# titus-leistner/mmlf

Measured on AMD Instinct MI355X. Metric: 96x96 EPI patches/sec fwd+bwd, bs=512, higher is better.
Workload: dtype f32 via 2 x f16 operand split (22 significant bits per operand, locally scaled; 3 MFMA passes, f32 accumulate)

## Files before the change

mmlf_amd/csrc/elementwise.hip:

```cpp
#include "common.h"
#include "row_walk.h"
#include "../../include/mmlf_hip.h"

thread_local char g_mmlf_err[512] = "";

extern "C" const char *mmlf_last_error(void) { return g_mmlf_err; }
extern "C" int mmlf_abi_version(void) { return MMLF_ABI_VERSION; }
extern "C" int64_t mmlf_amax_entries(int B, int H, int W)
{
    if (B <= 0 || H <= 0 || W <= 0) return -1;
    return amax_entries(make_grid(B, H, W));
}
extern "C" int mmlf_grid_pad_w(void) { return GRID_PAD; }
extern "C" int mmlf_grid_pad_h(void) { return GRID_PAD; }
extern "C" int mmlf_amax_head(void) { return MMLF_AMAX_HEAD; }
extern "C" int mmlf_amax_shard_stride(void) { return MMLF_AMAX_SHARD_STRIDE; }
extern "C" int64_t mmlf_grid_alloc_positions(int B, int H, int W)
{
    if (B <= 0 || H <= 0 || W <= 0) return -1;
    return grid_alloc_positions(make_grid(B, H, W));
}
extern "C" int64_t mmlf_grid_alloc_positions_k3(int B, int H, int W)
{
    if (B <= 0 || H <= 0 || W <= 0) return -1;
// ... 154 lines not shown
{
    double a = 0, b = 0;
    for (int blk = threadIdx.x; blk < nblocks; blk += 64) {
        a += partial[((size_t)blk * 2 + 0) * C + c];
        b += partial[((size_t)blk * 2 + 1) * C + c];
    }
    for (int off = 32; off > 0; off >>= 1) {
        a += __shfl_down(a, off, 64);
        b += __shfl_down(b, off, 64);
    }
    s0 = a; s1 = b;
}

__global__ __launch_bounds__(64) void bn_stats_finalize_kernel(const double *__restrict__ partial, int nblocks, int C,
                                                               double n, const float *__restrict__ gamma,
                                                               const float *__restrict__ beta, float *running_mean,
                                                               float *running_var, double momentum, double eps,
                                                               float *save_mean, float *save_invstd, float *scale,
                                                               float *shift)
{
    const int c = blockIdx.x;
    double s, ss;
    reduce_partials(partial, nblocks, C, c, s, ss);
    if (threadIdx.x != 0) return;
    const double mean = s / n;
    double var = ss / n - mean * mean;
    if (var < 0) var = 0;
    const double invstd = 1.0 / sqrt(var + eps);
    const float meanf = (float)mean, invf = (float)invstd;
    save_mean[c] = meanf;
    save_invstd[c] = invf;
    if (running_mean) {
        const double unb = n > 1 ? var * n / (n - 1) : var;
        running_mean[c] = (float)((1.0 - momentum) * running_mean[c] + momentum * mean);
        running_var[c] = (float)((1.0 - momentum) * running_var[c] + momentum * unb);
    }
    const float sc = (gamma ? gamma[c] : 1.f) * invf;
    scale[c] = sc;
    shift[c] = (beta ? beta[c] : 0.f) - meanf * sc;
}

__global__ void bn_coeffs_eval_kernel(const float *gamma, const float *beta, const float *rm, const float *rv,
                                      double eps, float *scale, float *shift, int C)
{
    const int c = blockIdx.x * blockDim.x + threadIdx.x;
    if (c >= C) return;
    const float sc = (float)((double)(gamma ? gamma[c] : 1.f) * (1.0 / sqrt((double)rv[c] + eps)));
    scale[c] = sc;
    shift[c] = fmaf(-rm[c], sc, beta ? beta[c] : 0.f);
}

__global__ __launch_bounds__(64) void bn_bwd_finalize_kernel(const double *__restrict__ partial, int nblocks, int C,
                                                             double n, const float *__restrict__ gamma,
                                                             const float *__restrict__ invstd, float *dgamma,
                                                             float *dbeta, int accumulate, float *coef)
{
    const int c = blockIdx.x;
    double sg, sgx;
    reduce_partials(partial, nblocks, C, c, sg, sgx);
    if (threadIdx.x != 0) return;
    if (dgamma) dgamma[c] = accumulate ? dgamma[c] + (float)sgx : (float)sgx;
    if (dbeta) dbeta[c] = accumulate ? dbeta[c] + (float)sg : (float)sg;
    const double k1 = (double)(gamma ? gamma[c] : 1.f) * invstd[c];
    coef[c] = (float)k1;
    coef[C + c] = (float)(k1 * sg / n);
    coef[2 * C + c] = (float)(k1 * (double)invstd[c] * sgx / n);
}

__global__ void fold_bn_kernel(const float *__restrict__ w, const float *__restrict__ b,
                               const float *__restrict__ scale, const float *__restrict__ shift,
                               float *__restrict__ w_out, float *__restrict__ b_out, int Cout, int per_co)
{
    const long long total = (long long)Cout * per_co;
    for (long long i = blockIdx.x * (long long)blockDim.x + threadIdx.x; i < total;
         i += (long long)gridDim.x * blockDim.x) {
        const int co = (int)(i / per_co);
        w_out[i] = w[i] * scale[co];
        if (i % per_co == 0) b_out[co] = fmaf(b ? b[co] : 0.f, scale[co], shift[co]);
    }
}

template <class Op>
__device__ __forceinline__ void for_each_row_pair(int cvn, int H, int W, int nrows, float *__restrict__ amax, Op op)
{
    const int P = W + GRID_PAD, R = H + GRID_PAD;
    const RowWalk w = row_walk(cvn);
    for (int row = blockIdx.x; row < nrows; row += gridDim.x) {
        const size_t base = (size_t)row * P;
        const bool row_in = grid_row_interior(row, R, H);
        float mx = 0.f;
        int x, cg;
        for (bool in = row_walk_start(w, threadIdx.x, P, x, cg); in; in = row_walk_step(w, P, x, cg))
            op(base + x, row_in && grid_pos_interior(x, W), cg, mx);
        if (amax) mmlf_amax_update_row(mx, amax, row);
    }
}

template <int MODE, int V>
__global__ __launch_bounds__(256) void bn_rows_kernel(const float *__restrict__ z, int cs_z,
                                                      const float *__restrict__ gy, int cs_gy, int c_off_gy,
                                                      const float *__restrict__ scale,
                                                      const float *__restrict__ shift,
                                                      const float *__restrict__ mean,
                                                      const float *__restrict__ coef, int C,
                                                      float *__restrict__ out, int cs_out, int c_off_out,
                                                      int C_store, int H, int W, float *__restrict__ amax, int nrows)
{
    extern __shared__ float coefs[];
    const int cvn = row_groups(C_store, V);
    const int Cpad = cvn * V;
    for (int c = threadIdx.x; c < Cpad; c += blockDim.x) {
        const bool ok = c < C;
        coefs[c] = ok ? scale[c] : 0.f;
        coefs[Cpad + c] = ok ? shift[c] : 0.f;
        if (MODE == 1) {
            coefs[2 * Cpad + c] = ok ? mean[c] : 0.f;
            coefs[3 * Cpad + c] = ok ? coef[c] : 0.f;
            coefs[4 * Cpad + c] = ok ? coef[C + c] : 0.f;
            coefs[5 * Cpad + c] = ok ? coef[2 * C + c] : 0.f;
        }
    }
    __syncthreads();
    for_each_row_pair(cvn, H, W, nrows, amax, [&](size_t q, bool interior, int cg, float &mx) {
        float o[V];
#pragma unroll
        for (int k = 0; k < V; ++k) o[k] = 0.f;
        if (interior && V * cg < C) {
            float zz[V], gg[V];
            VecIO<V>::load_nt(z + q * cs_z + V * cg, zz);
            if (MODE == 1) VecIO<V>::load_nt(gy + q * cs_gy + c_off_gy + V * cg, gg);
#pragma unroll
            for (int k = 0; k < V; ++k) {
                const int c = V * cg + k;
                const float u = fmaf(zz[k], coefs[c], coefs[Cpad + c]);
                if (MODE == 0) {
                    o[k] = fmaxf(u, 0.f);
                } else {
                    const float g = u > 0.f ? gg[k] : 0.f;
                    o[k] = coefs[3 * Cpad + c] * g - coefs[4 * Cpad + c] - coefs[5 * Cpad + c] * (zz[k] - coefs[2 * Cpad + c]);
                }
            }
        }
#pragma unroll
        for (int k = 0; k < V; ++k) mx = fmaxf(mx, fabsf(o[k]));
        float *op = out + q * cs_out + c_off_out + V * cg;
        if (V * cg + V - 1 < C_store) {
            VecIO<V>::store_nt(op, o);
        } else {
#pragma unroll
            for (int k = 0; k < V; ++k)
                if (V * cg + k < C_store) op[k] = o[k];
        }
    });
}

template <int V>
__global__ __launch_bounds__(256) void relu_slice_rows_kernel(const float *__restrict__ src, int cs_src, int c_off,
                                                              const float *__restrict__ ref, int cs_ref, int ref_off, int C,
                                                              float *__restrict__ dst, int cs_dst, int H, int W,
                                                              float *__restrict__ amax, int nrows)
{
    for_each_row_pair(cs_dst / V, H, W, nrows, amax, [&](size_t q, bool interior, int cg, float &mx) {
        float o[V];
#pragma unroll
        for (int k = 0; k < V; ++k) o[k] = 0.f;
        if (interior && V * cg < C) {
            const float *sp = src + q * cs_src + c_off + V * cg;
            const float *rp = ref + q * cs_ref + ref_off + V * cg;
            float rr[V];
            if (V * cg + V - 1 < C) {
                VecIO<V>::load_nt(sp, o);
                VecIO<V>::load_nt(rp, rr);
            } else {
#pragma unroll
                for (int k = 0; k < V; ++k) {
                    const bool in = V * cg + k < C;
                    o[k] = in ? sp[k] : 0.f;
                    rr[k] = in ? rp[k] : 0.f;
                }
            }
#pragma unroll
            for (int k = 0; k < V; ++k) o[k] = rr[k] > 0.f ? o[k] : 0.f;
        }
#pragma unroll
        for (int k = 0; k < V; ++k) mx = fmaxf(mx, fabsf(o[k]));
        VecIO<V>::store_nt(dst + q * cs_dst + V * cg, o);
    });
}

struct BnApply4 { const float *z[4]; const float *scale[4]; const float *shift[4]; };
__global__ __launch_bounds__(256) void bn_apply4_kernel(BnApply4 s, int cs_z, int C, float *__restrict__ out,
                                                        int H, int W, float *__restrict__ amax, int nrows)
{
    extern __shared__ float coefs[];
    const int C4 = 4 * C, half = C / 2;
    for (int c = threadIdx.x; c < C4; c += blockDim.x) {
        const int k = c / C, cl = c - k * C;
        const float *sc = k == 0 ? s.scale[0] : k == 1 ? s.scale[1] : k == 2 ? s.scale[2] : s.scale[3];
        const float *sh = k == 0 ? s.shift[0] : k == 1 ? s.shift[1] : k == 2 ? s.shift[2] : s.shift[3];
        coefs[c] = sc[cl];
        coefs[C4 + c] = sh[cl];
    }
    __syncthreads();
    for_each_row_pair(2 * C, H, W, nrows, amax, [&](size_t q, bool interior, int g, float &mx) {
        float2 o = make_float2(0.f, 0.f);
        if (interior) {
            const int k = g / half, cl = 2 * (g - k * half);
            const float *zp = k == 0 ? s.z[0] : k == 1 ? s.z[1] : k == 2 ? s.z[2] : s.z[3];
            const float2 zz = *reinterpret_cast<const float2 *>(zp + q * cs_z + cl);
            o.x = fmaxf(fmaf(zz.x, coefs[2 * g], coefs[C4 + 2 * g]), 0.f);
            o.y = fmaxf(fmaf(zz.y, coefs[2 * g + 1], coefs[C4 + 2 * g + 1]), 0.f);
        }
        mx = fmaxf(mx, fmaxf(o.x, o.y));
        *reinterpret_cast<float2 *>(out + q * C4 + 2 * g) = o;
    });
}


__global__ __launch_bounds__(256) void pack_nchw_kernel(const float *__restrict__ src, int C,
                                                        float *__restrict__ grid, int cs, int H, int W,
                                                        float *__restrict__ amax, int xt)
{
    extern __shared__ float tile[];
    float mx = 0.f;
    const int P = W + GRID_PAD, R = H + GRID_PAD;
    const int row = blockIdx.x;
    const int b = row / R, y = row - b * R;
    const size_t base = (size_t)row * P;
    const int c4n = cs / 4;
    const int pitch = xt | 1;
    const bool row_in = (y >= 1 && y <= H);
    for (int x0 = 0; x0 < P; x0 += xt) {
        const int nx = min(xt, P - x0);
        for (int e = threadIdx.x; e < cs * nx; e += blockDim.x) {
            const int c = e / nx, x = x0 + e - c * nx;
            float v = 0.f;
            if (row_in && x >= 1 && x <= W && c < C) v = src[(((size_t)b * C + c) * H + (y - 1)) * W + (x - 1)];
            tile[c * pitch + (x - x0)] = v;
        }
        __syncthreads();
        for (int e = threadIdx.x; e < nx * c4n; e += blockDim.x) {
            const int xl = e / c4n, cg = e - xl * c4n;
            const float4 o = make_float4(tile[(4 * cg) * pitch + xl], tile[(4 * cg + 1) * pitch + xl],
                                         tile[(4 * cg + 2) * pitch + xl], tile[(4 * cg + 3) * pitch + xl]);
            mx = fmaxf(fmaxf(mx, fmaxf(fabsf(o.x), fabsf(o.y))), fmaxf(fabsf(o.z), fabsf(o.w)));
            *reinterpret_cast<float4 *>(grid + (base + x0 + xl) * cs + 4 * cg) = o;
        }
        __syncthreads();
    }
    if (amax) mmlf_amax_update_row(mx, amax, row);
}

__global__ __launch_bounds__(256) void unpack_nchw_kernel(const float *__restrict__ grid, int cs,
                                                          float *__restrict__ dst, int C, int H, int W, int xt)
{
    extern __shared__ float tile[];
    const int P = W + GRID_PAD, R = H + GRID_PAD;
    const int row = blockIdx.x;
    const int b = row / H, y = row - b * H + 1;
    const size_t base = ((size_t)(b * R + y)) * P;
    const int pitch = C | 1;
    for (int x0 = 0; x0 < W; x0 += xt) {
        const int nx = min(xt, W - x0);
        for (int e = threadIdx.x; e < nx * C; e += blockDim.x) {
            const int xl = e / C, c = e - xl * C;
            tile[xl * pitch + c] = grid[(base + x0 + xl + 1) * cs + c];
        }
        __syncthreads();
        for (int e = threadIdx.x; e < C * nx; e += blockDim.x) {
            const int c = e / nx, xl = e - c * nx;
            dst[(((size_t)b * C + c) * H + (y - 1)) * W + x0 + xl] = tile[xl * pitch + c];
        }
        __syncthreads();
    }
}

__device__ __forceinline__ float laplace_pdf(float x, float mu, float b)
{
    const float a = __fdiv_rn(1.0f, __fmul_rn(2.0f, b));
    const float t = __fdiv_rn(-fabsf(__fsub_rn(x, mu)), b);
    return __fmul_rn(a, expf(t));
}

__global__ void head_upr_kernel(const float *__restrict__ out, const float *__restrict__ grid,
                                float *__restrict__ post, int steps, int HW, long long total)
{
    for (long long idx = blockIdx.x * (long long)blockDim.x + threadIdx.x; idx < total;
         idx += (long long)gridDim.x * blockDim.x) {
        const long long b = idx / HW;
        const int p = (int)(idx - b * HW);
        const float mu = out[(b * 2 + 0) * HW + p];
        const float bb = expf(out[(b * 2 + 1) * HW + p]);
        for (int k = 0; k < steps; ++k) post[(b * steps + k) * HW + p] = laplace_pdf(grid[k], mu, bb);
    }
}

__global__ void head_dpp_kernel(const float *__restrict__ sc, const float *__restrict__ gt, const float *__restrict__ gn,
                                float *__restrict__ one_hot, float *__restrict__ post, float *__restrict__ mean,
                                float *__restrict__ logvar, int steps, int HW, long long total)
{
    for (long long idx = blockIdx.x * (long long)blockDim.x + threadIdx.x; idx < total;
         idx += (long long)gridDim.x * blockDim.x) {
        const long long b = idx / HW;
        const int p = (int)(idx - b * HW);
        const float *s = sc + b * steps * HW + p;
        float mx = -INFINITY, z = 0.f;
// ... 674 lines not shown
        const int p = (int)(idx - b * HW);
        float best = INFINITY;
        int bi = 0;
        for (int j = 0; j < S; ++j) {
            const float lv = logvars[(size_t)j * total + idx];
            if (lv < best) { best = lv; bi = j; }
        }
        mean[idx] = means[(size_t)bi * total + idx];
        logvar[idx] = best;
        for (int k = 0; k < S; ++k) {
            const float gk = grid[k];
            float acc = 0.f;
            for (int j = 0; j < S; ++j)
                acc = __fadd_rn(acc, laplace_pdf(gk, means[(size_t)j * total + idx],
                                                 expf(logvars[(size_t)j * total + idx])));
            post[(b * S + k) * HW + p] = __fdiv_rn(acc, (float)S);
        }
    }
}

__device__ __forceinline__ double cdf_laplace_f64(double x, double m, double v)
{
    const double z = (x - m) / v;
    return x < m ? exp(z) / 2.0 : 1.0 - exp(-z) / 2.0;
}

__global__ void lmm_to_discrete_kernel(const float *__restrict__ means, const float *__restrict__ logvars,
                                       const double *__restrict__ edges, double *__restrict__ out, int S, int B,
                                       int n_bins, long long HW)
{
    const long long total = (long long)B * n_bins * HW;
    for (long long idx = blockIdx.x * (long long)blockDim.x + threadIdx.x; idx < total;
         idx += (long long)gridDim.x * blockDim.x) {
        const long long p = idx % HW;
        const long long r = idx / HW;
        const int k = (int)(r % n_bins);
        const long long b = r / n_bins;
        const double e0 = edges[k], e1 = edges[k + 1];
        double acc = 0.0;
        for (int s = 0; s < S; ++s) {
            const size_t o = ((size_t)s * B + b) * HW + p;
            const double m = (double)means[o];
            const double v = (double)expf(logvars[o]);
            acc += cdf_laplace_f64(e1, m, v) - cdf_laplace_f64(e0, m, v);
        }
        out[idx] = acc / (double)S;
    }
}

static int ew_blocks(long long total, int per = 256)
{
    long long b = (total + per - 1) / per;
    if (b > 8192) b = 8192;
    if (b < 1) b = 1;
    return (int)b;
}

extern "C" int mmlf_bn_stats_train(const float *z, int cs, int C, const float *gamma, const float *beta,
                                   float *running_mean, float *running_var, double momentum, double eps,
                                   float *save_mean, float *save_invstd, float *scale, float *shift,
                                   double *partial, int nblocks, int B, int H, int W, void *stream)
{
    MMLF_CHECK_ARG(z && save_mean && save_invstd && scale && shift && partial, "mmlf_bn_stats_train: null pointer");
    MMLF_CHECK_ARG(cs % 4 == 0 && C > 0 && C <= cs && (C + 3) / 4 <= 256, "mmlf_bn_stats_train: C=%d cs=%d", C, cs);
    MMLF_CHECK_ARG(nblocks > 0 && nblocks <= 4096, "mmlf_bn_stats_train: nblocks=%d", nblocks);
    MMLF_CHECK_ARG(B > 0 && H > 0 && W > 0, "mmlf_bn_stats_train: bad shape B=%d H=%d W=%d", B, H, W);
    hipStream_t st = (hipStream_t)stream;
    hipLaunchKernelGGL((bn_reduce_kernel<4>), dim3(nblocks), dim3(256), 0, st, z, cs, nullptr, 0, 0, nullptr,
                       nullptr, nullptr, nullptr, C, partial, B, H, W);
    const double n = (double)B * H * W;
    hipLaunchKernelGGL(bn_stats_finalize_kernel, dim3(C), dim3(64), 0, st, partial, nblocks, C, n, gamma,
                       beta, running_mean, running_var, momentum, eps, save_mean, save_invstd, scale, shift);
    return mmlf_launch_status("mmlf_bn_stats_train");
}

extern "C" int mmlf_bn_stats_finalize(const double *partial, int nblocks, int C, const float *gamma,
                                      const float *beta, float *running_mean, float *running_var, double momentum,
                                      double eps, float *save_mean, float *save_invstd, float *scale, float *shift,
                                      int B, int H, int W, void *stream)
{
    MMLF_CHECK_ARG(partial && save_mean && save_invstd && scale && shift && C > 0 && nblocks > 0,
                   "mmlf_bn_stats_finalize: bad argument");
    MMLF_CHECK_ARG(B > 0 && H > 0 && W > 0, "mmlf_bn_stats_finalize: bad shape B=%d H=%d W=%d", B, H, W);
    hipLaunchKernelGGL(bn_stats_finalize_kernel, dim3(C), dim3(64), 0, (hipStream_t)stream, partial, nblocks, C,
                       (double)B * H * W, gamma, beta, running_mean, running_var, momentum, eps, save_mean,
                       save_invstd, scale, shift);
    return mmlf_launch_status("mmlf_bn_stats_finalize");
}

extern "C" int mmlf_bn_coeffs_eval(const float *gamma, const float *beta, const float *rm, const float *rv,
                                   double eps, float *scale, float *shift, int C, void *stream)
{
    MMLF_CHECK_ARG(rm && rv && scale && shift && C > 0, "mmlf_bn_coeffs_eval: bad argument");
    hipLaunchKernelGGL(bn_coeffs_eval_kernel, dim3((C + 63) / 64), dim3(64), 0, (hipStream_t)stream, gamma, beta, rm,
                       rv, eps, scale, shift, C);
    return mmlf_launch_status("mmlf_bn_coeffs_eval");
}

static int fold_bn_eval(const char *who, int taps, const float *w_oihw, const float *bias, const float *scale,
                        const float *shift, float *w_out, float *bias_out, int Cout, int Cin, void *stream)
{
    MMLF_CHECK_ARG(w_oihw && scale && shift && w_out && bias_out && Cout > 0 && Cin > 0, "%s: bad argument", who);
    const long long total = (long long)Cout * Cin * taps;
    hipLaunchKernelGGL(fold_bn_kernel, dim3(ew_blocks(total)), dim3(256), 0, (hipStream_t)stream, w_oihw, bias, scale,
                       shift, w_out, bias_out, Cout, Cin * taps);
    return mmlf_launch_status(who);
}

extern "C" int mmlf_fold_bn_eval(const float *w_oihw, const float *bias, const float *scale, const float *shift,
                                 float *w_out, float *bias_out, int Cout, int Cin, void *stream)
{
    return fold_bn_eval("mmlf_fold_bn_eval", 4, w_oihw, bias, scale, shift, w_out, bias_out, Cout, Cin, stream);
}

extern "C" int mmlf_fold_bn_eval3x3(const float *w_oihw, const float *bias, const float *scale, const float *shift,
                                    float *w_out, float *bias_out, int Cout, int Cin, void *stream)
{
    return fold_bn_eval("mmlf_fold_bn_eval3x3", 9, w_oihw, bias, scale, shift, w_out, bias_out, Cout, Cin, stream);
}

extern "C" int mmlf_bn_apply_relu(const float *z, int cs_z, int C, const float *scale, const float *shift, float *y,
                                  int cs_y, int c_off, int C_store, int B, int H, int W, float *amax_out,
                                  void *stream)
{
    MMLF_CHECK_ARG(z && scale && shift && y, "mmlf_bn_apply_relu: null pointer");
    MMLF_CHECK_ARG(cs_z % 4 == 0 && cs_y % 2 == 0 && c_off % 2 == 0 && c_off >= 0 && C > 0 && C <= cs_z && C_store >= C &&
                       c_off + C_store <= cs_y,
                   "mmlf_bn_apply_relu: C=%d cs_z=%d cs_y=%d c_off=%d C_store=%d", C, cs_z, cs_y, c_off, C_store);
    MMLF_CHECK_ARG(B > 0 && H > 0 && W > 0, "mmlf_bn_apply_relu: bad shape B=%d H=%d W=%d", B, H, W);
    const int nrows = B * (H + GRID_PAD);
    hipLaunchKernelGGL((bn_rows_kernel<0, 4>), dim3(nrows), dim3(256), 6 * (C_store + 4) * sizeof(float), (hipStream_t)stream, z, cs_z,
                       nullptr, 0, 0, scale, shift, nullptr, nullptr, C, y, cs_y, c_off, C_store, H, W, amax_out, nrows);
    return mmlf_launch_status("mmlf_bn_apply_relu");
}

extern "C" int mmlf_bn_apply_relu4(const float *const z[4], int cs_z, int C, const float *const scale[4],
                                   const float *const shift[4], float *y, int cs_y, int B, int H, int W,
                                   float *amax_out, void *stream)
{
    MMLF_CHECK_ARG(z && scale && shift && y && B > 0 && H > 0 && W > 0, "mmlf_bn_apply_relu4: bad argument");
    MMLF_CHECK_ARG(C > 0 && C % 2 == 0 && C <= cs_z && cs_z % 2 == 0 && cs_y == 4 * C && 8 * C * sizeof(float) <= 48 * 1024,
                   "mmlf_bn_apply_relu4: C=%d cs_z=%d cs_y=%d (needs even C, cs_y == 4 * C)", C, cs_z, cs_y);
    BnApply4 s;
    for (int k = 0; k < 4; ++k) {
        MMLF_CHECK_ARG(z[k] && scale[k] && shift[k], "mmlf_bn_apply_relu4: null pointer in source %d", k);
        s.z[k] = z[k]; s.scale[k] = scale[k]; s.shift[k] = shift[k];
    }
    const int nrows = B * (H + GRID_PAD);
    hipLaunchKernelGGL(bn_apply4_kernel, dim3(nrows), dim3(256), 8 * C * sizeof(float), (hipStream_t)stream, s, cs_z, C,
                       y, H, W, amax_out, nrows);
    return mmlf_launch_status("mmlf_bn_apply_relu4");
}

extern "C" int mmlf_bn_bwd_reduce(const float *gy, int cs_gy, int c_off, const float *z, int cs_z, int C,
                                  const float *scale, const float *shift, const float *gamma,
                                  const float *save_mean, const float *save_invstd, float *dgamma, float *dbeta,
                                  int accumulate, float *coef, double *partial, int nblocks, int B, int H, int W,
                                  void *stream)
{
    MMLF_CHECK_ARG(gy && z && scale && shift && save_mean && save_invstd && coef && partial,
                   "mmlf_bn_bwd_reduce: null pointer");
    MMLF_CHECK_ARG(cs_gy % 2 == 0 && c_off % 2 == 0 && c_off >= 0 && cs_z % 4 == 0 && C > 0 && C <= cs_z &&
                       c_off + C <= cs_gy && (C + 3) / 4 <= 128,
                   "mmlf_bn_bwd_reduce: layout C=%d cs_z=%d cs_gy=%d c_off=%d", C, cs_z, cs_gy, c_off);
    MMLF_CHECK_ARG(nblocks > 0 && nblocks <= 4096, "mmlf_bn_bwd_reduce: nblocks=%d", nblocks);
    MMLF_CHECK_ARG(B > 0 && H > 0 && W > 0, "mmlf_bn_bwd_reduce: bad shape B=%d H=%d W=%d", B, H, W);
    hipStream_t st = (hipStream_t)stream;
    hipLaunchKernelGGL(bn_reduce_bwd_kernel, dim3(nblocks), dim3(256), 0, st, z, cs_z, gy, cs_gy, c_off,
                       scale, shift, save_mean, save_invstd, C, partial, B, H, W);
    hipLaunchKernelGGL(bn_bwd_finalize_kernel, dim3(C), dim3(64), 0, st, partial, nblocks, C,
                       (double)B * H * W, gamma, save_invstd, dgamma, dbeta, accumulate, coef);
    return mmlf_launch_status("mmlf_bn_bwd_reduce");
}

extern "C" int mmlf_bn_bwd_apply(const float *gy, int cs_gy, int c_off, const float *z, int cs_z, int C,
                                 const float *scale, const float *shift, const float *save_mean, const float *coef,
                                 float *dz, int cs_dz, int B, int H, int W, float *amax_out, void *stream)
{
    MMLF_CHECK_ARG(gy && z && scale && shift && save_mean && coef && dz, "mmlf_bn_bwd_apply: null pointer");
    MMLF_CHECK_ARG(cs_gy % 2 == 0 && c_off % 2 == 0 && c_off >= 0 && cs_z % 4 == 0 && cs_dz % 4 == 0 && C > 0 && C <= cs_z &&
                       C <= cs_dz && c_off + C <= cs_gy,
                   "mmlf_bn_bwd_apply: layout C=%d cs_z=%d cs_dz=%d cs_gy=%d c_off=%d", C, cs_z, cs_dz, cs_gy, c_off);
    MMLF_CHECK_ARG(B > 0 && H > 0 && W > 0, "mmlf_bn_bwd_apply: bad shape B=%d H=%d W=%d", B, H, W);
    const int nrows = B * (H + GRID_PAD);
    hipLaunchKernelGGL((bn_rows_kernel<1, 4>), dim3(nrows), dim3(256), 6 * (cs_dz + 4) * sizeof(float), (hipStream_t)stream, z, cs_z, gy,
                       cs_gy, c_off, scale, shift, save_mean, coef, C, dz, cs_dz, 0, cs_dz, H, W, amax_out, nrows);
    return mmlf_launch_status("mmlf_bn_bwd_apply");
}

static int relu_bwd_slice_args(const char *who, int cs_src, int c_off, int cs_ref, int ref_off, int C, int cs_dst, int B, int H,
                               int W)
{
    MMLF_CHECK_ARG(cs_src > 0 && cs_src % 2 == 0 && c_off % 2 == 0 && c_off >= 0 && cs_dst > 0 && cs_dst % 4 == 0 && C > 0 &&
                       C <= cs_dst && c_off + C <= cs_src && (C + 3) / 4 <= 128 && cs_dst / 4 <= 256,
                   "%s: layout C=%d cs_src=%d c_off=%d cs_dst=%d", who, C, cs_src, c_off, cs_dst);
    MMLF_CHECK_ARG(cs_ref > 0 && cs_ref % 2 == 0 && ref_off % 2 == 0 && ref_off >= 0 && ref_off + C <= cs_ref,
                   "%s: layout C=%d cs_ref=%d ref_off=%d", who, C, cs_ref, ref_off);
    MMLF_CHECK_ARG(B > 0 && H > 0 && W > 0, "%s: bad shape B=%d H=%d W=%d", who, B, H, W);
    return 0;
}

extern "C" int mmlf_relu_bwd_slice(const float *src, int cs_src, int c_off, const float *ref, int cs_ref, int ref_off, int C,
                                   float *dst, int cs_dst, int B, int H, int W, float *amax_out, void *stream)
{
    MMLF_CHECK_ARG(src && ref && dst, "mmlf_relu_bwd_slice: null pointer");
    if (relu_bwd_slice_args("mmlf_relu_bwd_slice", cs_src, c_off, cs_ref, ref_off, C, cs_dst, B, H, W)) return 1;
    const int nrows = B * (H + GRID_PAD);
    hipLaunchKernelGGL((relu_slice_rows_kernel<4>), dim3(nrows), dim3(256), 0, (hipStream_t)stream, src, cs_src, c_off, ref,
                       cs_ref, ref_off, C, dst, cs_dst, H, W, amax_out, nrows);
    return mmlf_launch_status("mmlf_relu_bwd_slice");
}

extern "C" int mmlf_audit_relu_bwd_slice(int cs_src, int c_off, int cs_ref, int ref_off, int C, int cs_dst, int B, int H, int W,
                                         int64_t *ends )
{
    MMLF_CHECK_ARG(ends, "mmlf_audit_relu_bwd_slice: null pointer");
    if (relu_bwd_slice_args("mmlf_audit_relu_bwd_slice", cs_src, c_off, cs_ref, ref_off, C, cs_dst, B, H, W)) return 1;
    const Grid g = make_grid(B, H, W);
    const long long q_last = ((long long)(B - 1) * g.R + H) * g.P + W;
    ends[MMLF_AUDIT_SLICE_SRC] = (q_last * cs_src + c_off + C) * 4;
    ends[MMLF_AUDIT_SLICE_REF] = (q_last * cs_ref + ref_off + C) * 4;
    ends[MMLF_AUDIT_SLICE_DST] = g.NQ * cs_dst * 4;
    ends[MMLF_AUDIT_SLICE_AMAX] = (MMLF_AMAX_HEAD + (long long)B * g.R) * 4;
    return 0;
}

extern "C" int mmlf_pack_nchw(const float *nchw, int C, float *grid, int cs, int B, int H, int W, float *amax_out,
                              void *stream)
{
    MMLF_CHECK_ARG(nchw && grid && C > 0 && cs % 4 == 0 && C <= cs, "mmlf_pack_nchw: C=%d cs=%d", C, cs);
    MMLF_CHECK_ARG(B > 0 && H > 0 && W > 0, "mmlf_pack_nchw: bad shape B=%d H=%d W=%d", B, H, W);
    const int xt = pack_tile_positions(cs);
    const size_t lds = (size_t)cs * (xt | 1) * sizeof(float);
    MMLF_CHECK_ARG(lds <= 64 * 1024, "mmlf_pack_nchw: cs=%d does not fit the transpose tile", cs);
    hipLaunchKernelGGL(pack_nchw_kernel, dim3(B * (H + GRID_PAD)), dim3(256), lds, (hipStream_t)stream, nchw, C, grid, cs, H, W,
                       amax_out, xt);
    return mmlf_launch_status("mmlf_pack_nchw");
}

__global__ void zero_slack_kernel(float *__restrict__ buf, long long head, long long tail_off, long long tail,
                                  float *__restrict__ amax, long long n_amax)
{
    for (long long i = blockIdx.x * (long long)blockDim.x + threadIdx.x; i < head + tail + n_amax;
         i += (long long)gridDim.x * blockDim.x) {
        if (i < head + tail) buf[i < head ? i : tail_off + (i - head)] = 0.f;
        else amax[i - head - tail] = 0.f;
    }
}

static int zero_slack_impl(float *grid, int cs, int B, int H, int W, float *amax, int ksize, void *stream)
{
    MMLF_CHECK_ARG(grid && cs > 0 && B > 0 && H > 0 && W > 0, "mmlf_zero_slack: bad argument");
    const Grid g = make_grid(B, H, W);
    const long long head = (long long)(g.P + 1) * cs, tail_off = g.NQ * cs;
    const long long tail = ((ksize == 3 ? grid_alloc_positions_k3(g) : grid_alloc_positions(g)) - g.NQ) * cs;
    const long long n_amax = amax ? amax_entries(g) : 0;
    hipLaunchKernelGGL(zero_slack_kernel, dim3(ew_blocks(head + tail + n_amax)), dim3(256), 0, (hipStream_t)stream, grid,
                       head, tail_off, tail, amax, n_amax);
    return mmlf_launch_status("mmlf_zero_slack");
}

extern "C" int mmlf_zero_slack(float *grid, int cs, int B, int H, int W, float *amax, void *stream)
{
    return zero_slack_impl(grid, cs, B, H, W, amax, 2, stream);
}

extern "C" int mmlf_zero_slack_k3(float *grid, int cs, int B, int H, int W, float *amax, void *stream)
{
    return zero_slack_impl(grid, cs, B, H, W, amax, 3, stream);
}

struct ZeroSlack4 { float *buf[4]; float *amax[4]; long long head[4], tail_off[4], tail[4], end[4]; long long n_amax; };
__global__ void zero_slack4_kernel(ZeroSlack4 z)
{
    for (long long i = blockIdx.x * (long long)blockDim.x + threadIdx.x; i < z.end[3]; i += (long long)gridDim.x * blockDim.x) {
        const int k = i < z.end[0] ? 0 : i < z.end[1] ? 1 : i < z.end[2] ? 2 : 3;
        const long long j = i - (k ? z.end[k - 1] : 0);
        if (j < z.head[k] + z.tail[k]) z.buf[k][j < z.head[k] ? j : z.tail_off[k] + (j - z.head[k])] = 0.f;
        else z.amax[k][j - z.head[k] - z.tail[k]] = 0.f;
    }
}

static int zero_slack4_impl(float *const grid[4], const int cs[4], float *const amax[4], int B, int H, int W, int ksize,
                            void *stream)
{
    MMLF_CHECK_ARG(grid && cs && amax && B > 0 && H > 0 && W > 0, "mmlf_zero_slack4: bad argument");
    const Grid g = make_grid(B, H, W);
    ZeroSlack4 z;
    long long run = 0;
    for (int k = 0; k < 4; ++k) {
        z.buf[k] = grid[k]; z.amax[k] = amax[k];
        z.head[k] = z.tail_off[k] = z.tail[k] = 0;
        if (grid[k]) {
            MMLF_CHECK_ARG(cs[k] > 0, "mmlf_zero_slack4: cs[%d]=%d", k, cs[k]);
            z.head[k] = (long long)(g.P + 1) * cs[k];
            z.tail_off[k] = g.NQ * cs[k];
            z.tail[k] = ((ksize == 3 ? grid_alloc_positions_k3(g) : grid_alloc_positions(g)) - g.NQ) * cs[k];
            run += z.head[k] + z.tail[k] + (amax[k] ? amax_entries(g) : 0);
        }
        z.end[k] = run;
    }
    z.n_amax = amax_entries(g);
    if (run == 0) return 0;
    hipLaunchKernelGGL(zero_slack4_kernel, dim3(ew_blocks(run)), dim3(256), 0, (hipStream_t)stream, z);
    return mmlf_launch_status("mmlf_zero_slack4");
}

extern "C" int mmlf_zero_slack4(float *const grid[4], const int cs[4], float *const amax[4], int B, int H, int W, void *stream)
{
    return zero_slack4_impl(grid, cs, amax, B, H, W, 2, stream);
}

extern "C" int mmlf_zero_slack4_k3(float *const grid[4], const int cs[4], float *const amax[4], int B, int H, int W,
                                   void *stream)
{
    return zero_slack4_impl(grid, cs, amax, B, H, W, 3, stream);
}

extern "C" int mmlf_unpack_nchw(const float *grid, int cs, float *nchw, int C, int B, int H, int W, void *stream)
{
    MMLF_CHECK_ARG(nchw && grid && C > 0 && C <= cs && cs % 4 == 0, "mmlf_unpack_nchw: C=%d cs=%d", C, cs);
    MMLF_CHECK_ARG(B > 0 && H > 0 && W > 0, "mmlf_unpack_nchw: bad shape B=%d H=%d W=%d", B, H, W);
    const int xt = unpack_tile_positions(C);
    hipLaunchKernelGGL(unpack_nchw_kernel, dim3(B * H), dim3(256), (size_t)xt * (C | 1) * sizeof(float), (hipStream_t)stream,
                       grid, cs, nchw, C, H, W, xt);
    return mmlf_launch_status("mmlf_unpack_nchw");
}

extern "C" int mmlf_head_upr(const float *output, const float *grid108, float *posterior, int steps, int B, int H,
                             int W, void *stream)
{
    MMLF_CHECK_ARG(output && grid108 && posterior && steps > 0, "mmlf_head_upr: bad argument");
    MMLF_CHECK_ARG(B > 0 && H > 0 && W > 0, "mmlf_head_upr: B=%d H=%d W=%d", B, H, W);
    const long long total = (long long)B * H * W;
    hipLaunchKernelGGL(head_upr_kernel, dim3(ew_blocks(total)), dim3(256), 0, (hipStream_t)stream, output, grid108,
                       posterior, steps, H * W, total);
    return mmlf_launch_status("mmlf_head_upr");
}

// ... 187 lines not shown
```

mmlf_amd/csrc/row_walk.h:

```cpp
#pragma once

constexpr int ROW_THREADS = 256;

__host__ __device__ __forceinline__ int row_groups(int c, int v) { return (c + v - 1) / v; }

struct RowWalk { int cvn, dx, dc; };
__host__ __device__ __forceinline__ RowWalk row_walk(int cvn)
{
    RowWalk w;
    w.cvn = cvn;
    w.dx = ROW_THREADS / cvn;
    w.dc = ROW_THREADS - w.dx * cvn;
    return w;
}
__host__ __device__ __forceinline__ bool row_walk_start(const RowWalk &w, int tid, int limit, int &x, int &cg)
{
    x = tid / w.cvn;
    cg = tid - x * w.cvn;
    return x < limit;
}
__host__ __device__ __forceinline__ bool row_walk_step(const RowWalk &w, int limit, int &x, int &cg)
{
    x += w.dx;
    cg += w.dc;
    if (cg >= w.cvn) { cg -= w.cvn; ++x; }
    return x < limit;
}

__host__ __device__ __forceinline__ bool grid_row_interior(int row, int R, int H)
{
    const int y = row % R;
    return y >= 1 && y <= H;
}
__host__ __device__ __forceinline__ bool grid_pos_interior(int x, int W) { return x >= 1 && x <= W; }

static inline int pack_tile_positions(int cs)
{
    int xt = 128;
    while (xt > 4 && (size_t)cs * (xt | 1) * sizeof(float) > 32 * 1024) xt >>= 1;
    return xt;
}
static inline int unpack_tile_positions(int C)
{
    int xt = 32;
    while (xt > 1 && (size_t)xt * (C | 1) * sizeof(float) > 32 * 1024) xt >>= 1;
    return xt;
}

__host__ __device__ __forceinline__ void reduce_walk(int C, int v, int &cvn, int &ppi)
{
    cvn = row_groups(C, v);
    ppi = ROW_THREADS / cvn;
}
```

Baseline: 1166.

## Stream BN backward reads through a per-wave LDS DMA ring with persistent blocks

Adds two persistent-grid kernels for the batch-norm backward pass, one for the reduction sums and one for the dz apply. They prefetch z and gy into a six-stage per-wave LDS ring using global_load_lds_dwordx4 DMA, so several loads stay in flight while earlier stages are being computed. The host launches them with a grid sized to the CU count and falls back to the old kernels when alignment or LDS limits are not met. This targets memory-latency stalls in these bandwidth-bound passes, at the cost of inline-asm m0/vmcnt handling, larger LDS use, and fewer resident blocks.

```diff
diff --git a/mmlf_amd/csrc/elementwise.hip b/mmlf_amd/csrc/elementwise.hip
--- a/mmlf_amd/csrc/elementwise.hip
+++ b/mmlf_amd/csrc/elementwise.hip
@@ -330,6 +330,216 @@
                 if (V * cg + k < C_store) op[k] = o[k];
         }
     });
+}
+
+typedef __attribute__((address_space(3))) void ew_lds_t;
+typedef float f4 __attribute__((ext_vector_type(4)));
+
+__device__ __forceinline__ void ring_dma16(const float *src, unsigned dst)
+{
+    unsigned keep;
+    asm volatile("s_mov_b32 %0, m0\n\ts_mov_b32 m0, %2\n\ts_nop 0\n\t"
+                 "global_load_lds_dwordx4 %1, off nt\n\ts_mov_b32 m0, %0"
+                 : "=&s"(keep) : "v"(src), "s"(dst) : "memory");
+}
+__device__ __forceinline__ void ring_wait_oldest() { asm volatile("s_waitcnt vmcnt(%0)" ::"n"(2 * (RING_STAGES - 1)) : "memory"); }
+__device__ __forceinline__ void ring_drain() { asm volatile("s_waitcnt vmcnt(0)" ::: "memory"); }
+__device__ __forceinline__ void ring_reads_done() { asm volatile("s_waitcnt lgkmcnt(0)" ::: "memory"); }
+
+__global__ __launch_bounds__(256)
+void bn_dz_stream_kernel(const float *__restrict__ z, int cs_z, const float *__restrict__ gy, int cs_gy, int c_off_gy,
+                         const float *__restrict__ scale, const float *__restrict__ shift, const float *__restrict__ mean,
+                         const float *__restrict__ coef, int C, float *__restrict__ out, int cs_out, int H, int W,
+                         float *__restrict__ amax, int nrows)
+{
+    extern __shared__ __attribute__((aligned(16))) unsigned char stream_lds[];
+    float *coefs = reinterpret_cast<float *>(stream_lds + RING_BYTES);
+    const int cvn = row_groups(cs_out, 4);
+    const int Cpad = cvn * 4;
+    const int tid = threadIdx.x;
+    for (int c = tid; c < Cpad; c += 256) {
+        const bool ok = c < C;
+        coefs[c] = ok ? scale[c] : 0.f;
+        coefs[Cpad + c] = ok ? shift[c] : 0.f;
+        coefs[2 * Cpad + c] = ok ? mean[c] : 0.f;
+        coefs[3 * Cpad + c] = ok ? coef[c] : 0.f;
+        coefs[4 * Cpad + c] = ok ? coef[C + c] : 0.f;
+        coefs[5 * Cpad + c] = ok ? coef[2 * C + c] : 0.f;
+    }
+    __syncthreads();
+    const int P = W + GRID_PAD, R = H + GRID_PAD;
+    const RowWalk w = row_walk(cvn);
+    const int steps = stream_row_steps(P, cvn);
+    const unsigned lds0 = (unsigned)(size_t)(ew_lds_t *)stream_lds;
+    const float *g0 = gy + c_off_gy;
+
+    int prow = blockIdx.x, pk = 0, pslot = 0, px, pcg;
+    bool prow_in = prow < nrows && grid_row_interior(prow, R, H);
+    row_walk_start(w, tid, P, px, pcg);
+    auto issue = [&]() {
+        const bool live = prow_in && grid_pos_interior(px, W) && 4 * pcg < C;
+        const size_t q = (size_t)prow * P + px;
+        const int wave = __builtin_amdgcn_readfirstlane(tid >> 6);
+        ring_dma16(live ? z + q * cs_z + 4 * pcg : z, lds0 + ring_piece(wave, pslot, 0));
+        ring_dma16(live ? g0 + q * cs_gy + 4 * pcg : g0, lds0 + ring_piece(wave, pslot, 1));
+        pslot = ring_next(pslot);
+        if (++pk == steps) {
+            pk = 0;
+            prow += gridDim.x;
+            prow_in = prow < nrows && grid_row_interior(prow, R, H);
+            row_walk_start(w, tid, P, px, pcg);
+        } else {
+            row_walk_step(w, P, px, pcg);
+        }
+    };
+    for (int s = 0; s < RING_STAGES; ++s) issue();
+
+    int crow = blockIdx.x, ck = 0, cslot = 0, cx, ccg;
+    bool crow_in = crow < nrows && grid_row_interior(crow, R, H);
+    row_walk_start(w, tid, P, cx, ccg);
+    float mx = 0.f;
+    while (crow < nrows) {
+        const f4 *kp = reinterpret_cast<const f4 *>(coefs + 4 * ccg);
+        const int kq = Cpad / 4;
+        const f4 sc = kp[0], sh = kp[kq];
+        ring_wait_oldest();
+        const f4 zv = *reinterpret_cast<const f4 *>(stream_lds + ring_cell(tid, cslot, 0));
+        const f4 gv = *reinterpret_cast<const f4 *>(stream_lds + ring_cell(tid, cslot, 1));
+        const f4 mu = kp[2 * kq], k1 = kp[3 * kq], k2 = kp[4 * kq], k3 = kp[5 * kq];
+        if (cx < P) {
+            float o[4];
+#pragma unroll
+            for (int k = 0; k < 4; ++k) o[k] = 0.f;
+            if (crow_in && grid_pos_interior(cx, W) && 4 * ccg < C) {
+#pragma unroll
+                for (int k = 0; k < 4; ++k) {
+                    const float u = fmaf(zv[k], sc[k], sh[k]);
+                    const float g = u > 0.f ? gv[k] : 0.f;
+                    o[k] = k1[k] * g - k2[k] - k3[k] * (zv[k] - mu[k]);
+                }
+            }
+#pragma unroll
+            for (int k = 0; k < 4; ++k) mx = fmaxf(mx, fabsf(o[k]));
+            const f4 ov = {o[0], o[1], o[2], o[3]};
+            __builtin_nontemporal_store(ov, reinterpret_cast<f4 *>(out + ((size_t)crow * P + cx) * cs_out + 4 * ccg));
+        }
+        ring_reads_done();
+        issue();
+        cslot = ring_next(cslot);
+        if (++ck == steps) {
+            if (amax) mmlf_amax_update_row(mx, amax, crow);
+            mx = 0.f;
+            ck = 0;
+            crow += gridDim.x;
+            crow_in = crow < nrows && grid_row_interior(crow, R, H);
+            row_walk_start(w, tid, P, cx, ccg);
+        } else {
+            row_walk_step(w, P, cx, ccg);
+        }
+    }
+    ring_drain();
+}
+
+__global__ __launch_bounds__(256)
+void bn_sums_stream_kernel(const float *__restrict__ z, int cs_z, const float *__restrict__ gy, int cs_gy, int c_off,
+                           const float *__restrict__ scale, const float *__restrict__ shift, const float *__restrict__ mean,
+                           const float *__restrict__ invstd, int C, double *__restrict__ partial, int nblocks, int B, int H, int W)
+{
+    extern __shared__ __attribute__((aligned(16))) unsigned char stream_lds[];
+    static_assert(2 * 256 * 4 * sizeof(double) <= RING_BYTES, "the block's sums fit the ring");
+    double *red = reinterpret_cast<double *>(stream_lds);
+    float *cf = reinterpret_cast<float *>(stream_lds + RING_BYTES);
+    const int P = W + GRID_PAD, R = H + GRID_PAD;
+    int cvn, ppi;
+    reduce_walk(C, 4, cvn, ppi);
+    const int Cpad = cvn * 4;
+    const int tid = threadIdx.x;
+    const int pl = tid / cvn, cg = tid - pl * cvn;
+    const bool active = pl < ppi;
+    for (int c = tid; c < Cpad; c += 256) {
+        const bool in = c < C;
+        float *k = cf + 4 * ((c & 3) * SUMS_GROUPS + (c >> 2));
+        k[0] = in ? scale[c] : 0.f;
+        k[1] = in ? shift[c] : 0.f;
+        k[2] = in ? mean[c] : 0.f;
+        k[3] = in ? invstd[c] : 0.f;
+    }
+    const int nrows = B * H;
+    const int steps = reduce_row_steps(W, ppi);
+    const unsigned lds0 = (unsigned)(size_t)(ew_lds_t *)stream_lds;
+    const float *g0 = gy + c_off;
+    for (int v = blockIdx.x; v < nblocks; v += gridDim.x) {
+        __syncthreads();
+        double s0[4], s1[4];
+#pragma unroll
+        for (int e = 0; e < 4; ++e) { s0[e] = 0; s1[e] = 0; }
+        if (v < nrows) {
+            int prow = v, pk = 0, pslot = 0;
+            size_t pbase = 0;
+            auto row_base = [&](int row) {
+                const int b = row / H, y = row - b * H + 1;
+                return (size_t)(b * R + y) * P + 1;
+            };
+            pbase = row_base(prow);
+            auto issue = [&]() {
+                const int x = pl + pk * ppi;
+                const bool live = active && x < W && prow < nrows;
+                const int wave = __builtin_amdgcn_readfirstlane(tid >> 6);
+                ring_dma16(live ? z + (pbase + x) * cs_z + 4 * cg : z, lds0 + ring_piece(wave, pslot, 0));
+                ring_dma16(live ? g0 + (pbase + x) * cs_gy + 4 * cg : g0, lds0 + ring_piece(wave, pslot, 1));
+                pslot = ring_next(pslot);
+                if (++pk == steps) {
+                    pk = 0;
+                    prow += nblocks;
+                    if (prow < nrows) pbase = row_base(prow);
+                }
+            };
+            for (int s = 0; s < RING_STAGES; ++s) issue();
+            int ck = 0, cslot = 0;
+            for (int crow = v; crow < nrows;) {
+                const f4 *kp = reinterpret_cast<const f4 *>(cf + 4 * cg);
+                f4 k = kp[0];
+                ring_wait_oldest();
+                const f4 zv = *reinterpret_cast<const f4 *>(stream_lds + ring_cell(tid, cslot, 0));
+                const f4 gv = *reinterpret_cast<const f4 *>(stream_lds + ring_cell(tid, cslot, 1));
+                const bool mine = active && pl + ck * ppi < W;
+                if (mine) {
+#pragma unroll
+                    for (int e = 0; e < 4; ++e) {
+                        f4 kn = k;
+                        if (e < 3) kn = kp[(e + 1) * SUMS_GROUPS];
+                        const float u = fmaf(zv[e], k[0], k[1]);
+                        const float g = u > 0.f ? gv[e] : 0.f;
+                        s0[e] += g;
+                        s1[e] += (double)g * (double)((zv[e] - k[2]) * k[3]);
+                        asm volatile("" : "+v"(s1[e]) : : "memory");
+                        k = kn;
+                    }
+                }
+                ring_reads_done();
+                issue();
+                cslot = ring_next(cslot);
+                if (++ck == steps) { ck = 0; crow += nblocks; }
+            }
+            ring_drain();
+            __syncthreads();
+        }
+#pragma unroll
+        for (int e = 0; e < 4; ++e) { red[(0 * 256 + tid) * 4 + e] = s0[e]; red[(1 * 256 + tid) * 4 + e] = s1[e]; }
+        __syncthreads();
+        if (tid < cvn) {
+#pragma unroll
+            for (int e = 0; e < 4; ++e) {
+                double a0 = 0, a1 = 0;
+                for (int p = 0; p < ppi; ++p) { a0 += red[(0 * 256 + p * cvn + tid) * 4 + e]; a1 += red[(1 * 256 + p * cvn + tid) * 4 + e]; }
+                const int c = 4 * tid + e;
+                if (c < C) {
+                    partial[((size_t)v * 2 + 0) * C + c] = a0;
+                    partial[((size_t)v * 2 + 1) * C + c] = a1;
+                }
+            }
+        }
+    }
 }
 
 template <int V>
@@ -1310,6 +1520,22 @@
     return mmlf_launch_status("mmlf_bn_apply_relu4");
 }
 
+static bool stream_sources_ok(const float *z, const float *gy, int cs_gy, int c_off)
+{
+    return (reinterpret_cast<uintptr_t>(z) & 15) == 0 && (reinterpret_cast<uintptr_t>(gy + c_off) & 15) == 0 && cs_gy % 4 == 0;
+}
+static int stream_blocks()
+{
+    static int blocks[64] = {};
+    const int dev = current_device();
+    if (!blocks[dev]) {
+        int n = 0;
+        if (hipDeviceGetAttribute(&n, hipDeviceAttributeMultiprocessorCount, dev) != hipSuccess || n <= 0) n = 256;
+        blocks[dev] = n / 8 * 8 < 8 ? 8 : n / 8 * 8;
+    }
+    return blocks[dev];
+}
+
 extern "C" int mmlf_bn_bwd_reduce(const float *gy, int cs_gy, int c_off, const float *z, int cs_z, int C,
                                   const float *scale, const float *shift, const float *gamma,
                                   const float *save_mean, const float *save_invstd, float *dgamma, float *dbeta,
@@ -1319,13 +1545,21 @@
     MMLF_CHECK_ARG(gy && z && scale && shift && save_mean && save_invstd && coef && partial,
                    "mmlf_bn_bwd_reduce: null pointer");
     MMLF_CHECK_ARG(cs_gy % 2 == 0 && c_off % 2 == 0 && c_off >= 0 && cs_z % 4 == 0 && C > 0 && C <= cs_z &&
-                       c_off + C <= cs_gy && (C + 3) / 4 <= 128,
+                       c_off + C <= cs_gy && (C + 3) / 4 <= SUMS_GROUPS,
                    "mmlf_bn_bwd_reduce: layout C=%d cs_z=%d cs_gy=%d c_off=%d", C, cs_z, cs_gy, c_off);
     MMLF_CHECK_ARG(nblocks > 0 && nblocks <= 4096, "mmlf_bn_bwd_reduce: nblocks=%d", nblocks);
     MMLF_CHECK_ARG(B > 0 && H > 0 && W > 0, "mmlf_bn_bwd_reduce: bad shape B=%d H=%d W=%d", B, H, W);
     hipStream_t st = (hipStream_t)stream;
-    hipLaunchKernelGGL(bn_reduce_bwd_kernel, dim3(nblocks), dim3(256), 0, st, z, cs_z, gy, cs_gy, c_off,
-                       scale, shift, save_mean, save_invstd, C, partial, B, H, W);
+    const int lds = stream_lds_bytes(4, SUMS_GROUPS, 4);
+    static_assert(stream_lds_bytes(4, SUMS_GROUPS, 4) <= STREAM_LDS_MAX, "the sums kernel's LDS");
+    if (stream_sources_ok(z, gy, cs_gy, c_off)) {
+        const int grid = nblocks < stream_blocks() ? nblocks : stream_blocks();
+        hipLaunchKernelGGL(bn_sums_stream_kernel, dim3(grid), dim3(256), lds, st, z, cs_z, gy, cs_gy, c_off, scale, shift,
+                           save_mean, save_invstd, C, partial, nblocks, B, H, W);
+    } else {
+        hipLaunchKernelGGL(bn_reduce_bwd_kernel, dim3(nblocks), dim3(256), 0, st, z, cs_z, gy, cs_gy, c_off,
+                           scale, shift, save_mean, save_invstd, C, partial, B, H, W);
+    }
     hipLaunchKernelGGL(bn_bwd_finalize_kernel, dim3(C), dim3(64), 0, st, partial, nblocks, C,
                        (double)B * H * W, gamma, save_invstd, dgamma, dbeta, accumulate, coef);
     return mmlf_launch_status("mmlf_bn_bwd_reduce");
@@ -1341,8 +1575,16 @@
                    "mmlf_bn_bwd_apply: layout C=%d cs_z=%d cs_dz=%d cs_gy=%d c_off=%d", C, cs_z, cs_dz, cs_gy, c_off);
     MMLF_CHECK_ARG(B > 0 && H > 0 && W > 0, "mmlf_bn_bwd_apply: bad shape B=%d H=%d W=%d", B, H, W);
     const int nrows = B * (H + GRID_PAD);
-    hipLaunchKernelGGL((bn_rows_kernel<1, 4>), dim3(nrows), dim3(256), 6 * (cs_dz + 4) * sizeof(float), (hipStream_t)stream, z, cs_z, gy,
-                       cs_gy, c_off, scale, shift, save_mean, coef, C, dz, cs_dz, 0, cs_dz, H, W, amax_out, nrows);
+    const int lds = stream_lds_bytes(6, cs_dz / 4, 4);
+    if (stream_sources_ok(z, gy, cs_gy, c_off) && (reinterpret_cast<uintptr_t>(dz) & 15) == 0 && lds <= STREAM_LDS_MAX &&
+        (long long)(W + GRID_PAD) * (cs_dz / 4) < (1ll << 30)) {
+        const int grid = nrows < stream_blocks() ? nrows : stream_blocks();
+        hipLaunchKernelGGL(bn_dz_stream_kernel, dim3(grid), dim3(256), lds, (hipStream_t)stream, z, cs_z, gy, cs_gy, c_off, scale,
+                           shift, save_mean, coef, C, dz, cs_dz, H, W, amax_out, nrows);
+    } else {
+        hipLaunchKernelGGL((bn_rows_kernel<1, 4>), dim3(nrows), dim3(256), 6 * (cs_dz + 4) * sizeof(float), (hipStream_t)stream, z, cs_z,
+                           gy, cs_gy, c_off, scale, shift, save_mean, coef, C, dz, cs_dz, 0, cs_dz, H, W, amax_out, nrows);
+    }
     return mmlf_launch_status("mmlf_bn_bwd_apply");
 }
 
diff --git a/mmlf_amd/csrc/row_walk.h b/mmlf_amd/csrc/row_walk.h
--- a/mmlf_amd/csrc/row_walk.h
+++ b/mmlf_amd/csrc/row_walk.h
@@ -52,3 +52,26 @@
     cvn = row_groups(C, v);
     ppi = ROW_THREADS / cvn;
 }
+
+constexpr int RING_STAGES = 6;
+constexpr int RING_PIECE_BYTES = 64 * 16;
+constexpr int RING_STAGE_BYTES = 2 * RING_PIECE_BYTES;
+constexpr int RING_WAVE_BYTES = RING_STAGES * RING_STAGE_BYTES;
+constexpr int RING_BYTES = (ROW_THREADS / 64) * RING_WAVE_BYTES;
+__host__ __device__ __forceinline__ int ring_next(int slot) { return slot + 1 == RING_STAGES ? 0 : slot + 1; }
+__host__ __device__ __forceinline__ unsigned ring_piece(int wave, int slot, int which)
+{
+    return (unsigned)(wave * RING_WAVE_BYTES + slot * RING_STAGE_BYTES + which * RING_PIECE_BYTES);
+}
+__host__ __device__ __forceinline__ unsigned ring_cell(int tid, int slot, int which)
+{
+    return ring_piece(tid >> 6, slot, which) + 16u * (unsigned)(tid & 63);
+}
+__host__ __device__ __forceinline__ int stream_row_steps(int limit, int cvn) { return (limit * cvn + ROW_THREADS - 1) / ROW_THREADS; }
+__host__ __device__ __forceinline__ int reduce_row_steps(int W, int ppi) { return (W + ppi - 1) / ppi; }
+constexpr int STREAM_LDS_MAX = 56 * 1024;
+constexpr int SUMS_GROUPS = 128;
+__host__ __device__ constexpr int stream_lds_bytes(int coefs_per_channel, int cvn, int v)
+{
+    return RING_BYTES + coefs_per_channel * cvn * v * (int)sizeof(float);
+}
```

New measurement: 1175 (median of 6 runs). No clear change (+0.8%).
